# DmitryUlyanov/deep-image-prior

Hardware: AMD Instinct MI355X
Metric: optimisation iters/sec per image (skip-net 512x512 denoising) (higher is better)
Workload: dtype f32

## Files before the change

deep-image-prior_amd/csrc/bf3.h:

```cpp
#pragma once
#include "dip_common.h"

typedef __bf16 bf16x8 __attribute__((ext_vector_type(8)));
typedef unsigned u32x2 __attribute__((ext_vector_type(2)));
typedef unsigned u32x4 __attribute__((ext_vector_type(4)));

__device__ __forceinline__ void dip_bf3_split(float a, unsigned& h, unsigned& m, unsigned& l) {
    const unsigned uh = __float_as_uint(a) & 0xFFFF0000u;
    const float r1 = a - __uint_as_float(uh);
    const unsigned um = __float_as_uint(r1) & 0xFFFF0000u;
    const float r2 = r1 - __uint_as_float(um);
    h = uh;
    m = um;
    l = __float_as_uint(r2) & 0xFFFF0000u;
}

__device__ __forceinline__ unsigned dip_bf3_pack2(unsigned x0, unsigned x1) { return (x0 >> 16) | x1; }
__device__ __forceinline__ u32x2 dip_bf3_pack4(const unsigned (&x)[4]) {
    return u32x2{dip_bf3_pack2(x[0], x[1]), dip_bf3_pack2(x[2], x[3])};
}

template <int TR>
__device__ __forceinline__ f32x4 dip_bf3_transform(f32x4 v, const float* a4p, const float* b4p, float slope) {
    if constexpr (TR != 0) {
        const f32x4 a4 = *reinterpret_cast<const f32x4*>(a4p), b4 = *reinterpret_cast<const f32x4*>(b4p);
#pragma unroll
        for (int e = 0; e < 4; ++e) {
            const float tv = fmaf(a4[e], v[e], b4[e]);
            v[e] = TR == 1 ? dip_act_leaky(tv, slope) : dip_act(tv, slope);
        }
    }
    return v;
}

template <int NT, class F>
__device__ __forceinline__ void dip_bf3_products(F&& f) {
    dip_static_for<0, 5>([&](auto S) {
        constexpr int sm = 4 - decltype(S)::value;
        if constexpr (!((NT == 6 && sm > 2) || (NT == 8 && sm > 3))) {
            dip_static_for<0, 3>([&](auto PA) {
                constexpr int pa = decltype(PA)::value, pb = sm - pa;
                if constexpr (pb >= 0 && pb <= 2) f(PA, std::integral_constant<int, pb>{});
            });
        }
    });
}

static inline int dip_bf3_tr(const DipTransform& tr) { return tr.a == nullptr ? 0 : (tr.slope > 0.f ? 1 : 2); }
template <class F>
int dip_bf3_dispatch(int nt, int tr, F&& f) {
    auto with_nt = [&](auto NT) {
        if (tr == 0) return f(NT, std::integral_constant<int, 0>{});
        if (tr == 1) return f(NT, std::integral_constant<int, 1>{});
        return f(NT, std::integral_constant<int, 2>{});
    };
    if (nt == 6) return with_nt(std::integral_constant<int, 6>{});
    if (nt == 8) return with_nt(std::integral_constant<int, 8>{});
    return with_nt(std::integral_constant<int, 9>{});
}
```

deep-image-prior_amd/csrc/wgrad_bf3.hip:

```cpp
#include "dip_common.h"
#include "dip_group.h"
#include "bf3.h"
#include <stdlib.h>

namespace {

#ifdef DIP_W3_PROFILE
__device__ unsigned long long g_w3_prof[1024 * 8 * 8];
__device__ int g_w3_mode;
#define W3_T() __builtin_amdgcn_s_memtime()
#define W3_ADD(slot, t0, t1) prof[slot] += (t1) - (t0)
#else
#define W3_T() 0ull
#define W3_ADD(slot, t0, t1) ((void)0)
#endif

struct W3Cfg {
    static constexpr int TH = 2, TW = 16;
    static constexpr int HTH = TH + 2, HTW = TW + 2;
    static constexpr int U_ROW = 48;
    static constexpr int U_CH = HTH * U_ROW + 16;
    static constexpr int U_PLANE = 32 * U_CH;
    static constexpr int D_ROW = 32;
    static constexpr int D_CH = TH * D_ROW + 16;
    static constexpr int D_PLANE = 128 * D_CH;
    static constexpr int U_PAIRS = HTH * 9 * 8;
    static constexpr int D_PAIRS = TH * 8 * 32;
    static constexpr int U_SLOTS = 2, D_SLOTS = 2;
    static constexpr int LDS_BYTES = 3 * U_PLANE + 3 * D_PLANE + 2 * 512 * 4;
};

__device__ __forceinline__ void w3_store_planes(unsigned char* base, const unsigned (&h)[2][4], const unsigned (&m)[2][4], const unsigned (&l)[2][4],
                                                int ch_pitch, int plane_pitch) {
#pragma unroll
    for (int e = 0; e < 4; ++e) {
        *reinterpret_cast<unsigned*>(base + e * ch_pitch) = dip_bf3_pack2(h[0][e], h[1][e]);
        *reinterpret_cast<unsigned*>(base + e * ch_pitch + plane_pitch) = dip_bf3_pack2(m[0][e], m[1][e]);
        *reinterpret_cast<unsigned*>(base + e * ch_pitch + 2 * plane_pitch) = dip_bf3_pack2(l[0][e], l[1][e]);
    }
}
template <int NT>
__device__ __forceinline__ void w3_taps_of_row(const u32x4 (&w0)[3], const unsigned (&w1)[3], const bf16x8 (&b)[3], f32x16& acc0,
                                               f32x16& acc1, f32x16& acc2) {
    bf16x8 a[3][3];
#pragma unroll
    for (int p = 0; p < 3; ++p) {
        a[0][p] = __builtin_bit_cast(bf16x8, w0[p]);
        a[1][p] = __builtin_bit_cast(bf16x8, u32x4{__builtin_amdgcn_alignbyte(w0[p][1], w0[p][0], 2), __builtin_amdgcn_alignbyte(w0[p][2], w0[p][1], 2),
                                                     __builtin_amdgcn_alignbyte(w0[p][3], w0[p][2], 2), __builtin_amdgcn_alignbyte(w1[p], w0[p][3], 2)});
        a[2][p] = __builtin_bit_cast(bf16x8, u32x4{w0[p][1], w0[p][2], w0[p][3], w1[p]});
    }
    dip_bf3_products<NT>([&](auto PA, auto PB) {
        constexpr int pa = decltype(PA)::value, pb = decltype(PB)::value;
        acc0 = __builtin_amdgcn_mfma_f32_32x32x16_bf16(a[0][pa], b[pb], acc0, 0, 0, 0);
        __builtin_amdgcn_sched_barrier(0x7F6);
        acc1 = __builtin_amdgcn_mfma_f32_32x32x16_bf16(a[1][pa], b[pb], acc1, 0, 0, 0);
        __builtin_amdgcn_sched_barrier(0x7F6);
        acc2 = __builtin_amdgcn_mfma_f32_32x32x16_bf16(a[2][pa], b[pb], acc2, 0, 0, 0);
        __builtin_amdgcn_sched_barrier(0x7F6);
    });
}

template <int NT, int TR>
__global__ __launch_bounds__(256, 2) void wgrad_bf3_v1_kernel(const DipWgradDesc d, const int ntx, const int ntiles, const int CinP,
                                                              const int CoutP) {
    using C = W3Cfg;
    extern __shared__ __attribute__((aligned(16))) unsigned char smem[];
    unsigned char* Us = smem;
    unsigned char* Ds = smem + 3 * C::U_PLANE;
    float* tra = reinterpret_cast<float*>(Ds + 3 * C::D_PLANE);
    float* trb = tra + 512;

    const int tid = threadIdx.x, lane = tid & 63, l31 = lane & 31, half = lane >> 5;
    const int wave = __builtin_amdgcn_readfirstlane(tid >> 6);
    const int walker = blockIdx.x, nwalk = gridDim.x;
    const int c0 = blockIdx.y * 32;
    const int o0 = blockIdx.z * 128;
    const bool wave_active = (o0 + wave * 32) < CoutP;
    const bool do_bias = d.bias_partial != nullptr && blockIdx.y == 0;
    const float slope = d.tr.slope;

    if (TR) {
        for (int c = tid; c < 32; c += 256) {
            const bool ok = c0 + c < d.Cin;
            tra[c] = ok ? d.tr.a[c0 + c] : 1.f;
            trb[c] = ok ? d.tr.b[c0 + c] : 0.f;
        }
    }
    for (int i = tid; i < (3 * C::U_PLANE + 3 * C::D_PLANE) / 4; i += 256) reinterpret_cast<unsigned*>(smem)[i] = 0u;

    f32x16 acc[9];
#pragma unroll
    for (int t = 0; t < 9; ++t)
#pragma unroll
        for (int r = 0; r < 16; ++r) acc[t][r] = 0.f;
    float bs[2][4] = {{0.f, 0.f, 0.f, 0.f}, {0.f, 0.f, 0.f, 0.f}};

    f32x4 ur[C::U_SLOTS][2], dr[C::D_SLOTS][2];
    auto fetch = [&](int tile) {
        const int ty = tile / ntx, tx = tile - ty * ntx;
#pragma unroll
        for (int i = 0; i < C::U_SLOTS; ++i) {
            const int s = tid + i * 256;
            const int cg = s / 36, rem = s - cg * 36, hr = rem / 9, pp = rem - hr * 9;
            const int c = c0 + cg * 4;
            const int sr = dip_map_src(ty * C::TH + hr - d.off, d.Hin, d.pad_mode);
            const bool okc = s < C::U_PAIRS && c < d.Cin && sr >= 0;
#pragma unroll
            for (int q = 0; q < 2; ++q) {
                const int sc = dip_map_src(tx * C::TW + 2 * pp + q - d.off, d.Win, d.pad_mode);
                const bool ok = okc && sc >= 0;
                ur[i][q] = *reinterpret_cast<const f32x4*>(d.x + ((size_t)(ok ? sr : 0) * d.Win + (ok ? sc : 0)) * d.Cx + (ok ? c : 0));
            }
        }
#pragma unroll
        for (int i = 0; i < C::D_SLOTS; ++i) {
            const int s = tid + i * 256;
            const int cg = s >> 4, rem = s & 15, r = rem >> 3, pp = rem & 7;
            const int o = o0 + cg * 4;
            const int oy = ty * C::TH + r;
#pragma unroll
            for (int q = 0; q < 2; ++q) {
                const int ox = tx * C::TW + 2 * pp + q;
                const bool ok = oy < d.Hout && ox < d.Wout && o < d.Cdy;
                dr[i][q] = *reinterpret_cast<const f32x4*>(d.dy + ((size_t)(ok ? oy : 0) * d.Wout + (ok ? ox : 0)) * d.Cdy + (ok ? o : 0));
            }
        }
    };
    auto commit = [&](int tile) {
        const int ty = tile / ntx, tx = tile - ty * ntx;
#pragma unroll
        for (int i = 0; i < C::U_SLOTS; ++i) {
            const int s = tid + i * 256;
            if (s < C::U_PAIRS) {
                const int cg = s / 36, rem = s - cg * 36, hr = rem / 9, pp = rem - hr * 9;
                const int c = c0 + cg * 4;
                const int sr = dip_map_src(ty * C::TH + hr - d.off, d.Hin, d.pad_mode);
                unsigned h[2][4], m[2][4], l[2][4];
#pragma unroll
                for (int q = 0; q < 2; ++q) {
                    const int sc = dip_map_src(tx * C::TW + 2 * pp + q - d.off, d.Win, d.pad_mode);
                    const bool ok = c < d.Cin && sr >= 0 && sc >= 0;
                    f32x4 v = ur[i][q];
                    if (TR) {
                        const f32x4 a4 = *reinterpret_cast<const f32x4*>(tra + cg * 4), b4 = *reinterpret_cast<const f32x4*>(trb + cg * 4);
#pragma unroll
                        for (int e = 0; e < 4; ++e) {
                            const float tv = fmaf(a4[e], v[e], b4[e]);
                            v[e] = TR == 1 ? dip_act_leaky(tv, slope) : dip_act(tv, slope);
                        }
                    }
#pragma unroll
                    for (int e = 0; e < 4; ++e) dip_bf3_split(ok ? v[e] : 0.f, h[q][e], m[q][e], l[q][e]);
                }
                w3_store_planes(Us + (cg * 4) * C::U_CH + hr * C::U_ROW + pp * 4, h, m, l, C::U_CH, C::U_PLANE);
            }
        }
#pragma unroll
        for (int i = 0; i < C::D_SLOTS; ++i) {
            const int s = tid + i * 256;
            const int cg = s >> 4, rem = s & 15, r = rem >> 3, pp = rem & 7;
            const int o = o0 + cg * 4;
            const int oy = ty * C::TH + r;
            unsigned h[2][4], m[2][4], l[2][4];
#pragma unroll
            for (int q = 0; q < 2; ++q) {
                const int ox = tx * C::TW + 2 * pp + q;
                const bool ok = oy < d.Hout && ox < d.Wout && o < d.Cdy;
#pragma unroll
                for (int e = 0; e < 4; ++e) {
                    const float v = ok ? dr[i][q][e] : 0.f;
                    bs[i][e] += v;
                    dip_bf3_split(v, h[q][e], m[q][e], l[q][e]);
                }
            }
            w3_store_planes(Ds + (cg * 4) * C::D_CH + r * C::D_ROW + pp * 4, h, m, l, C::D_CH, C::D_PLANE);
        }
    };

    const unsigned char* ua = Us + l31 * C::U_CH + 16 * half;
    const unsigned char* da = Ds + (wave * 32 + l31) * C::D_CH + 16 * half;

    __syncthreads();
    if (walker < ntiles) fetch(walker);
    for (int tile = walker; tile < ntiles; tile += nwalk) {
        __syncthreads();
        commit(tile);
        __syncthreads();
        if (tile + nwalk < ntiles) fetch(tile + nwalk);
        if (wave_active) {
#pragma unroll
            for (int s = 0; s < 2; ++s) {
                bf16x8 b[3];
#pragma unroll
                for (int p = 0; p < 3; ++p) b[p] = *reinterpret_cast<const bf16x8*>(da + p * C::D_PLANE + s * C::D_ROW);
#pragma unroll
                for (int ky = 0; ky < 3; ++ky) {
                    const int hr = s + ky;
                    u32x4 w0[3];
                    unsigned w1[3];
#pragma unroll
                    for (int p = 0; p < 3; ++p) {
                        w0[p] = *reinterpret_cast<const u32x4*>(ua + p * C::U_PLANE + hr * C::U_ROW);
                        w1[p] = *reinterpret_cast<const unsigned*>(ua + p * C::U_PLANE + hr * C::U_ROW + 16);
                    }
#pragma unroll
                    for (int kx = 0; kx < 3; ++kx) {
                        bf16x8 a[3];
#pragma unroll
                        for (int p = 0; p < 3; ++p) {
                            u32x4 v;
                            if (kx == 0) v = w0[p];
                            else if (kx == 2) v = u32x4{w0[p][1], w0[p][2], w0[p][3], w1[p]};
                            else v = u32x4{__builtin_amdgcn_alignbyte(w0[p][1], w0[p][0], 2), __builtin_amdgcn_alignbyte(w0[p][2], w0[p][1], 2),
                                           __builtin_amdgcn_alignbyte(w0[p][3], w0[p][2], 2), __builtin_amdgcn_alignbyte(w1[p], w0[p][3], 2)};
                            a[p] = __builtin_bit_cast(bf16x8, v);
                        }
                        const int t = ky * 3 + kx;
                        dip_bf3_products<NT>([&](auto PA, auto PB) {
                            acc[t] = __builtin_amdgcn_mfma_f32_32x32x16_bf16(a[decltype(PA)::value], b[decltype(PB)::value], acc[t], 0, 0, 0);
                        });
                    }
                    __builtin_amdgcn_sched_barrier(0);
                }
            }
        }
    }

    if (wave_active) {
        const int o = o0 + wave * 32 + l31;
#pragma unroll
        for (int t = 0; t < 9; ++t)
#pragma unroll
            for (int r = 0; r < 16; ++r) {
                const int c = c0 + (r & 3) + 8 * (r >> 2) + 4 * half;
                if (c < CinP) d.partial[(((size_t)walker * 9 + t) * CinP + c) * CoutP + o] = acc[t][r];
            }
    }
    if (do_bias) {
        __syncthreads();
        float* red = reinterpret_cast<float*>(smem);
#pragma unroll
        for (int i = 0; i < C::D_SLOTS; ++i)
#pragma unroll
            for (int e = 0; e < 4; ++e) red[(tid + i * 256) * 4 + e] = bs[i][e];
        __syncthreads();
        if (tid < 128 && o0 + tid < CoutP) {
            const int cg = tid >> 2, e = tid & 3;
            float sum = 0.f;
            for (int k = 0; k < 16; ++k) sum += red[(cg * 16 + k) * 4 + e];
            d.bias_partial[(size_t)walker * CoutP + o0 + tid] = sum;
        }
    }
}

template <int NT, int TR>
int w3_launch_v1(const DipWgradDesc& d, hipStream_t st) {
    using C = W3Cfg;
    auto kern = wgrad_bf3_v1_kernel<NT, TR>;
    static bool attr_set[16] = {};
    if (dip_once_per_device(attr_set)) {
        hipError_t e = hipFuncSetAttribute(reinterpret_cast<const void*>(kern), hipFuncAttributeMaxDynamicSharedMemorySize, 160 * 1024);
        if (e != hipSuccess) { dip_set_error(hipGetErrorString(e)); return (int)e; }
    }
    const int ntx = dip_cdiv(d.Wout, C::TW), nty = dip_cdiv(d.Hout, C::TH);
    const int CinP = dip_round_up(d.Cin, 32), CoutP = dip_round_up(d.Cout, 32);
    const int nfull = ((d.Cin & 31) >= 1 && (d.Cin & 31) <= 4 && d.Cin > 32) ? (d.Cin >> 5) : dip_cdiv(d.Cin, 32);
    dip_launch(kern, dim3(d.nsplit, nfull, dip_cdiv(CoutP, 128)), dim3(256), C::LDS_BYTES, st, d, ntx, ntx * nty, CinP, CoutP);
    DIP_CHECK_LAUNCH();
    return 0;
}


template <int NT, int TR>
__global__ __launch_bounds__(512) void wgrad_bf3_kernel(const DipWgradDesc d, const int ntx, const int ntiles, const int CinP,
                                                        const int CoutP, const int c_end) {
    using C = W3Cfg;
    constexpr int U_PLANE2 = 64 * C::U_CH;
    constexpr int BUF = 3 * U_PLANE2 + 3 * C::D_PLANE;
    extern __shared__ __attribute__((aligned(16))) unsigned char smem[];
    float* tra = reinterpret_cast<float*>(smem + 2 * BUF);
    float* trb = tra + 64;

    const int tid = threadIdx.x, lane = tid & 63, l31 = lane & 31, half = lane >> 5;
    const int wave = __builtin_amdgcn_readfirstlane(tid >> 6);
    const int grp = wave >> 2, wq = wave & 3, tg = tid & 255;
    const int walker = blockIdx.x, nwalk = gridDim.x;
    const int c0 = blockIdx.y * 64 + grp * 32;
    const int o0 = blockIdx.z * 128;
    const bool wave_active = (o0 + wq * 32) < CoutP;
    const bool do_bias = d.bias_partial != nullptr && blockIdx.y == 0;
    const float slope = d.tr.slope;

    if (TR) {
        if (tid < 64) {
            const int c = blockIdx.y * 64 + tid;
            const bool ok = c < d.Cin;
            tra[tid] = ok ? d.tr.a[c] : 1.f;
            trb[tid] = ok ? d.tr.b[c] : 0.f;
        }
    }
    for (int i = tid; i < 2 * BUF / 4; i += 512) reinterpret_cast<unsigned*>(smem)[i] = 0u;

    f32x16 acc[9];
#pragma unroll
    for (int t = 0; t < 9; ++t)
#pragma unroll
        for (int r = 0; r < 16; ++r) acc[t][r] = 0.f;
    float bs[4] = {0.f, 0.f, 0.f, 0.f};

    int u_off[2], u_lds[2], u_hr[2], u_pp[2];
    bool u_valid[2];
#pragma unroll
    for (int i = 0; i < 2; ++i) {
        const int s = tg + i * 256;
        const int cg = s & 7, rem = s >> 3, hr = rem / 9, pp = rem - hr * 9;
        u_hr[i] = hr;
        u_pp[i] = pp;
        u_valid[i] = s < C::U_PAIRS && (c0 + cg * 4) < d.Cin;
        u_off[i] = u_valid[i] ? (hr * d.Win + 2 * pp) * d.Cx + c0 + cg * 4 : 0;
        u_lds[i] = (grp * 32 + cg * 4) * C::U_CH + hr * C::U_ROW + pp * 4;
    }
    const int u_c = c0 + (tg & 7) * 4;
    const int d_pp = tid & 7, d_r = (tid >> 6) & 1, d_cg = ((tid >> 7) << 3) | ((tid >> 3) & 7);
    const int d_o = o0 + d_cg * 4;
    const bool d_valid = d_o < d.Cdy;
    const int d_off = d_valid ? (d_r * d.Wout + 2 * d_pp) * d.Cdy + d_o : 0;
    const int d_lds = 3 * U_PLANE2 + (d_cg * 4) * C::D_CH + d_r * C::D_ROW + d_pp * 4;
    auto interior = [&](int ty, int tx) {
        return ty * C::TH - d.off >= 0 && ty * C::TH + C::HTH - 1 - d.off < d.Hin && tx * C::TW - d.off >= 0 &&
               tx * C::TW + C::HTW - 1 - d.off < d.Win && ty * C::TH + C::TH - 1 < d.Hout && tx * C::TW + C::TW - 1 < d.Wout;
    };

    f32x4 ur[2][2], dr[2];
    auto fetch = [&](int tile) {
        const int ty = tile / ntx, tx = tile - ty * ntx;
        const float* pu[2][2];
        const float* pd[2];
        if (interior(ty, tx)) {
            const float* bx = d.x + ((size_t)(ty * C::TH - d.off) * d.Win + (tx * C::TW - d.off)) * d.Cx;
            const float* by = d.dy + ((size_t)(ty * C::TH) * d.Wout + tx * C::TW) * d.Cdy;
#pragma unroll
            for (int i = 0; i < 2; ++i) {
                pu[i][0] = bx + u_off[i];
                pu[i][1] = pu[i][0] + d.Cx;
            }
            pd[0] = by + d_off;
            pd[1] = pd[0] + d.Cdy;
        } else {
#pragma unroll
            for (int i = 0; i < 2; ++i) {
                const int sr = dip_map_src(ty * C::TH + u_hr[i] - d.off, d.Hin, d.pad_mode);
                const bool okc = u_valid[i] && sr >= 0;
#pragma unroll
                for (int q = 0; q < 2; ++q) {
                    const int sc = dip_map_src(tx * C::TW + 2 * u_pp[i] + q - d.off, d.Win, d.pad_mode);
                    const bool ok = okc && sc >= 0;
                    pu[i][q] = d.x + ((size_t)(ok ? sr : 0) * d.Win + (ok ? sc : 0)) * d.Cx + (ok ? u_c : 0);
                }
            }
            const int oy = ty * C::TH + d_r;
#pragma unroll
            for (int q = 0; q < 2; ++q) {
                const int ox = tx * C::TW + 2 * d_pp + q;
                const bool ok = oy < d.Hout && ox < d.Wout && d_valid;
                pd[q] = d.dy + ((size_t)(ok ? oy : 0) * d.Wout + (ok ? ox : 0)) * d.Cdy + (ok ? d_o : 0);
            }
        }
#pragma unroll
        for (int i = 0; i < 2; ++i)
#pragma unroll
            for (int q = 0; q < 2; ++q) ur[i][q] = *reinterpret_cast<const f32x4*>(pu[i][q]);
#pragma unroll
        for (int q = 0; q < 2; ++q) dr[q] = *reinterpret_cast<const f32x4*>(pd[q]);
    };
    auto commit = [&](int tile, int buf) {
        const int ty = tile / ntx, tx = tile - ty * ntx;
        unsigned char* Bs = smem + buf * BUF;
        bool oku[2][2], okd[2];
        if (interior(ty, tx)) {
#pragma unroll
            for (int i = 0; i < 2; ++i) oku[i][0] = oku[i][1] = u_valid[i];
            okd[0] = okd[1] = d_valid;
        } else {
#pragma unroll
            for (int i = 0; i < 2; ++i) {
                const int sr = dip_map_src(ty * C::TH + u_hr[i] - d.off, d.Hin, d.pad_mode);
#pragma unroll
                for (int q = 0; q < 2; ++q) {
                    const int sc = dip_map_src(tx * C::TW + 2 * u_pp[i] + q - d.off, d.Win, d.pad_mode);
                    oku[i][q] = u_valid[i] && sr >= 0 && sc >= 0;
                }
            }
            const int oy = ty * C::TH + d_r;
#pragma unroll
            for (int q = 0; q < 2; ++q) okd[q] = oy < d.Hout && (tx * C::TW + 2 * d_pp + q) < d.Wout && d_valid;
        }
#pragma unroll
        for (int i = 0; i < 2; ++i) {
            if (tg + i * 256 < C::U_PAIRS) {
                unsigned h[2][4], m[2][4], l[2][4];
#pragma unroll
                for (int q = 0; q < 2; ++q) {
                    f32x4 v = ur[i][q];
                    v = dip_bf3_transform<TR>(v, tra + grp * 32 + (tg & 7) * 4, trb + grp * 32 + (tg & 7) * 4, slope);
#pragma unroll
                    for (int e = 0; e < 4; ++e) dip_bf3_split(oku[i][q] ? v[e] : 0.f, h[q][e], m[q][e], l[q][e]);
                }
                w3_store_planes(Bs + u_lds[i], h, m, l, C::U_CH, U_PLANE2);
            }
        }
        {
            unsigned h[2][4], m[2][4], l[2][4];
#pragma unroll
            for (int q = 0; q < 2; ++q) {
#pragma unroll
                for (int e = 0; e < 4; ++e) {
                    const float v = okd[q] ? dr[q][e] : 0.f;
                    bs[e] += v;
                    dip_bf3_split(v, h[q][e], m[q][e], l[q][e]);
                }
            }
            w3_store_planes(Bs + d_lds, h, m, l, C::D_CH, C::D_PLANE);
        }
    };

    const int ua_off = (grp * 32 + l31) * C::U_CH + 16 * half;
    const int da_off = 3 * U_PLANE2 + (wq * 32 + l31) * C::D_CH + 16 * half;
    auto mfma_tile = [&](int buf) {
        const unsigned char* ua = smem + buf * BUF + ua_off;
        const unsigned char* da = smem + buf * BUF + da_off;
        bf16x8 b[2][3];
#pragma unroll
        for (int s = 0; s < 2; ++s)
#pragma unroll
            for (int p = 0; p < 3; ++p) b[s][p] = *reinterpret_cast<const bf16x8*>(da + p * C::D_PLANE + s * C::D_ROW);
        u32x4 w0[2][3];
        unsigned w1[2][3];
#pragma unroll
        for (int p = 0; p < 3; ++p) {
            w0[0][p] = *reinterpret_cast<const u32x4*>(ua + p * U_PLANE2);
            w1[0][p] = *reinterpret_cast<const unsigned*>(ua + p * U_PLANE2 + 16);
        }
#pragma unroll
        for (int hr = 0; hr < 4; ++hr) {
            const int cur = hr & 1, nxt = cur ^ 1;
            if (hr < 3) {
#pragma unroll
                for (int p = 0; p < 3; ++p) {
                    w0[nxt][p] = *reinterpret_cast<const u32x4*>(ua + p * U_PLANE2 + (hr + 1) * C::U_ROW);
                    w1[nxt][p] = *reinterpret_cast<const unsigned*>(ua + p * U_PLANE2 + (hr + 1) * C::U_ROW + 16);
                }
            }
#pragma unroll
            for (int s = 0; s < 2; ++s) {
                const int ky = hr - s;
                if (ky < 0 || ky > 2) continue;
                w3_taps_of_row<NT>(w0[cur], w1[cur], b[s], acc[ky * 3], acc[ky * 3 + 1], acc[ky * 3 + 2]);
            }
            __builtin_amdgcn_sched_barrier(0);
        }
    };

#ifdef DIP_W3_PROFILE
    unsigned long long prof[8] = {0, 0, 0, 0, 0, 0, 0, 0};
#endif
    const unsigned long long tk0 = W3_T();
#ifdef DIP_W3_PROFILE
    const unsigned long long tr0 = __builtin_amdgcn_s_memrealtime();
    const int w3_mode = __builtin_amdgcn_readfirstlane(g_w3_mode);
#else
    constexpr int w3_mode = 0;
#endif
    __syncthreads();
    const int ntl = walker < ntiles ? (ntiles - 1 - walker) / nwalk + 1 : 0;
    if (ntl > 0) {
        fetch(walker);
        commit(walker, 0);
        if (ntl > 1) fetch(walker + nwalk);
    }
    __syncthreads();
    for (int h = 0; h < 2 * ntl; ++h) {
        const int kt = h >> 1, buf = kt & 1;
        const unsigned long long t0 = W3_T();
        if ((h & 1) == grp) {
            if (wave_active && w3_mode != 1) {
                __builtin_amdgcn_s_setprio(2);
                mfma_tile(buf);
                __builtin_amdgcn_s_setprio(0);
            }
            const unsigned long long t1 = W3_T();
            __syncthreads();
            W3_ADD(0, t0, t1);
            W3_ADD(1, t1, W3_T());
        } else {
            unsigned long long t1 = t0, t2 = t0;
            if (kt + 1 < ntl && w3_mode != 2) {
                commit(walker + (kt + 1) * nwalk, buf ^ 1);
                t1 = W3_T();
                if (kt + 2 < ntl) fetch(walker + (kt + 2) * nwalk);
                t2 = W3_T();
            }
            __syncthreads();
            W3_ADD(2, t0, t1);
            W3_ADD(3, t1, t2);
            W3_ADD(4, t2, W3_T());
        }
#ifdef DIP_W3_PROFILE
        prof[5] += 1;
#endif
    }
#ifdef DIP_W3_PROFILE
    prof[6] = W3_T() - tk0;
    prof[7] = __builtin_amdgcn_s_memrealtime() - tr0;
    if (lane == 0) {
        const int wg = (blockIdx.z * gridDim.y + blockIdx.y) * gridDim.x + blockIdx.x;
        if (wg < 1024)
            for (int i = 0; i < 8; ++i) g_w3_prof[(wg * 8 + wave) * 8 + i] = prof[i];
    }
#endif

    if (wave_active && c0 < c_end) {
        const int o = o0 + wq * 32 + l31;
#pragma unroll
        for (int t = 0; t < 9; ++t)
#pragma unroll
            for (int r = 0; r < 16; ++r) {
                const int c = c0 + (r & 3) + 8 * (r >> 2) + 4 * half;
                if (c < CinP) d.partial[(((size_t)walker * 9 + t) * CinP + c) * CoutP + o] = acc[t][r];
            }
    }
    if (do_bias) {
        float* red = reinterpret_cast<float*>(smem);
#pragma unroll
        for (int e = 0; e < 4; ++e) red[tid * 4 + e] = bs[e];
        __syncthreads();
        if (tid < 128 && o0 + tid < CoutP) {
            const int cg = tid >> 2, e = tid & 3;
            float sum = 0.f;
            for (int k = 0; k < 16; ++k) sum += red[((k & 7) + 8 * (cg & 7) + 64 * (k >> 3) + 128 * (cg >> 3)) * 4 + e];
            d.bias_partial[(size_t)walker * CoutP + o0 + tid] = sum;
        }
    }
}

template <int NT, int TR>
int w3_launch(const DipWgradDesc& d, hipStream_t st) {
    using C = W3Cfg;
    constexpr int LDS2 = 2 * (3 * 64 * C::U_CH + 3 * C::D_PLANE) + 2 * 64 * 4;
    auto kern = wgrad_bf3_kernel<NT, TR>;
    static bool attr_set[16] = {};
    if (dip_once_per_device(attr_set)) {
        hipError_t e = hipFuncSetAttribute(reinterpret_cast<const void*>(kern), hipFuncAttributeMaxDynamicSharedMemorySize, 160 * 1024);
        if (e != hipSuccess) { dip_set_error(hipGetErrorString(e)); return (int)e; }
    }
    const int ntx = dip_cdiv(d.Wout, C::TW), nty = dip_cdiv(d.Hout, C::TH);
    const int CinP = dip_round_up(d.Cin, 32), CoutP = dip_round_up(d.Cout, 32);
    const int nfull = ((d.Cin & 31) >= 1 && (d.Cin & 31) <= 4 && d.Cin > 32) ? (d.Cin >> 5) : dip_cdiv(d.Cin, 32);
    const bool has_tail = (d.Cin & 31) >= 1 && (d.Cin & 31) <= 4 && d.Cin > 32;
    dip_launch(kern, dim3(d.nsplit, dip_cdiv(nfull, 2), dip_cdiv(CoutP, 128)), dim3(512), LDS2, st, d, ntx, ntx * nty, CinP, CoutP,
               has_tail ? nfull * 32 : CinP);
    DIP_CHECK_LAUNCH();
    return 0;
}

}

#ifdef DIP_W3_PROFILE
extern "C" int dip_w3_prof_mode(int mode) { return (int)hipMemcpyToSymbol(HIP_SYMBOL(g_w3_mode), &mode, sizeof(int)); }
extern "C" int dip_w3_prof_read(unsigned long long* host, int n) {
    return (int)hipMemcpyFromSymbol(host, HIP_SYMBOL(g_w3_prof), (size_t)n * sizeof(unsigned long long));
}
#endif

extern "C" int dip_conv_bf3_terms(void);
extern "C" int dip_conv_wgrad_tail(const DipWgradDesc* dp, void* stream);

extern "C" int dip_wgrad_bf3_eligible(const DipWgradDesc* dp) {
    const DipWgradDesc& d = *dp;
    static const bool off = getenv("DIP_WGRAD_NO_BF3") != nullptr;
    if (off || dip_conv_bf3_terms() == 0) return 0;
    if (d.ks != 3 || d.stride != 1 || d.Cin < 32 || d.Cout < 97 || d.tap_groups > 1) return 0;
    if ((d.Cx & 3) || (d.Cdy & 3) || (d.tr.a != nullptr && d.Cin > 512)) return 0;
    const int tail = d.Cin & 31;
    if (tail >= 1 && tail <= 4 && (d.Cin >> 5) > 8) return 0;
    const int ntiles = dip_cdiv(d.Wout, 16) * dip_cdiv(d.Hout, 2);
    if (d.nsplit < 1 || d.nsplit > dip_cdiv(d.Wout, 16) * dip_cdiv(d.Hout, 4)) return 0;
    return ntiles >= 512 ? 1 : 0;
}

extern "C" int dip_wgrad_bf3(const DipWgradDesc* dp, void* stream) {
    const DipWgradDesc& d = *dp;
    hipStream_t st = reinterpret_cast<hipStream_t>(stream);
    const int nt = dip_conv_bf3_terms();
    if (nt == 0) DIP_FAIL("wgrad_bf3: the bf16-pipe arithmetic is switched off (DIP_CONV_BF3=0)");
    static const int v1_mode = [] { const char* e = getenv("DIP_WGRAD_BF3_V1"); return e ? atoi(e) : 0; }();
    const bool v1 = v1_mode == 1 || (v1_mode == 2 && dip_cdiv(d.Wout, 16) * dip_cdiv(d.Hout, 2) < 2048);
    const int rc = dip_bf3_dispatch(nt, dip_bf3_tr(d.tr), [&](auto NT, auto TR) {
        constexpr int T = decltype(NT)::value, R = decltype(TR)::value;
        return v1 ? w3_launch_v1<T, R>(d, st) : w3_launch<T, R>(d, st);
    });
    if (rc) return rc;
    if ((d.Cin & 31) >= 1 && (d.Cin & 31) <= 4 && d.Cin > 32) return dip_conv_wgrad_tail(dp, stream);
    return 0;
}
```

Baseline: 184.7.

## Restructure wgrad bf3 staging: recompute slot indices, split halo row loads, use perm packing

The staging of x and dy tiles into LDS is reorganised. The old two-iteration loop, which left lanes idle on the halo, is replaced by one full f32x4 slot per thread plus a scalar 'mini' slot that loads the last halo row on waves 2 and up. Per-thread slot offsets are now recomputed in each fetch and commit behind an asm barrier, so they are not held in registers across the MFMA loop. Offsets become 32-bit byte offsets, with a new eligibility guard against overflow. bf16 packing now uses v_perm, and the low term's mask is dropped because perm selects only the upper bytes. This aims to cut register pressure and VALU work in the staging path, at the cost of repeated index arithmetic.

```diff
diff --git a/deep-image-prior_amd/csrc/bf3.h b/deep-image-prior_amd/csrc/bf3.h
--- a/deep-image-prior_amd/csrc/bf3.h
+++ b/deep-image-prior_amd/csrc/bf3.h
@@ -12,14 +12,45 @@
     const float r2 = r1 - __uint_as_float(um);
     h = uh;
     m = um;
-    l = __float_as_uint(r2) & 0xFFFF0000u;
+    l = __float_as_uint(r2);
+}
+__device__ __forceinline__ void dip_bf3_split2(f32x2 a, u32x2& h, u32x2& m, u32x2& l) {
+#pragma unroll
+    for (int e = 0; e < 2; ++e) {
+        unsigned he, me, le;
+        dip_bf3_split(a[e], he, me, le);
+        h[e] = he;
+        m[e] = me;
+        l[e] = le;
+    }
+}
+__device__ __forceinline__ void dip_bf3_split4(f32x4 a, u32x4& h, u32x4& m, u32x4& l) {
+#pragma unroll
+    for (int e = 0; e < 4; ++e) {
+        unsigned he, me, le;
+        dip_bf3_split(a[e], he, me, le);
+        h[e] = he;
+        m[e] = me;
+        l[e] = le;
+    }
 }
 
-__device__ __forceinline__ unsigned dip_bf3_pack2(unsigned x0, unsigned x1) { return (x0 >> 16) | x1; }
+__device__ __forceinline__ unsigned dip_bf3_pack2(unsigned x0, unsigned x1) { return __builtin_amdgcn_perm(x1, x0, 0x07060302u); }
 __device__ __forceinline__ u32x2 dip_bf3_pack4(const unsigned (&x)[4]) {
     return u32x2{dip_bf3_pack2(x[0], x[1]), dip_bf3_pack2(x[2], x[3])};
 }
 
+template <int TR>
+__device__ __forceinline__ f32x2 dip_bf3_transform2(f32x2 v, f32x2 a2, f32x2 b2, float slope) {
+    if constexpr (TR != 0) {
+#pragma unroll
+        for (int e = 0; e < 2; ++e) {
+            const float tv = fmaf(a2[e], v[e], b2[e]);
+            v[e] = TR == 1 ? dip_act_leaky(tv, slope) : dip_act(tv, slope);
+        }
+    }
+    return v;
+}
 template <int TR>
 __device__ __forceinline__ f32x4 dip_bf3_transform(f32x4 v, const float* a4p, const float* b4p, float slope) {
     if constexpr (TR != 0) {
diff --git a/deep-image-prior_amd/csrc/wgrad_bf3.hip b/deep-image-prior_amd/csrc/wgrad_bf3.hip
--- a/deep-image-prior_amd/csrc/wgrad_bf3.hip
+++ b/deep-image-prior_amd/csrc/wgrad_bf3.hip
@@ -38,6 +38,19 @@
         *reinterpret_cast<unsigned*>(base + e * ch_pitch + plane_pitch) = dip_bf3_pack2(m[0][e], m[1][e]);
         *reinterpret_cast<unsigned*>(base + e * ch_pitch + 2 * plane_pitch) = dip_bf3_pack2(l[0][e], l[1][e]);
     }
+}
+__device__ __forceinline__ void w3_store_planes(unsigned char* base, const u32x4 (&h)[2], const u32x4 (&m)[2], const u32x4 (&l)[2], int ch_pitch,
+                                                int plane_pitch) {
+#pragma unroll
+    for (int e = 0; e < 4; ++e) {
+        *reinterpret_cast<unsigned*>(base + e * ch_pitch) = dip_bf3_pack2(h[0][e], h[1][e]);
+        *reinterpret_cast<unsigned*>(base + e * ch_pitch + plane_pitch) = dip_bf3_pack2(m[0][e], m[1][e]);
+        *reinterpret_cast<unsigned*>(base + e * ch_pitch + 2 * plane_pitch) = dip_bf3_pack2(l[0][e], l[1][e]);
+    }
+}
+__device__ __forceinline__ unsigned w3_here(unsigned v) {
+    asm volatile("" : "+v"(v));
+    return v;
 }
 template <int NT>
 __device__ __forceinline__ void w3_taps_of_row(const u32x4 (&w0)[3], const unsigned (&w1)[3], const bf16x8 (&b)[3], f32x16& acc0,
@@ -309,119 +322,145 @@
         for (int r = 0; r < 16; ++r) acc[t][r] = 0.f;
     float bs[4] = {0.f, 0.f, 0.f, 0.f};
 
-    int u_off[2], u_lds[2], u_hr[2], u_pp[2];
-    bool u_valid[2];
-#pragma unroll
-    for (int i = 0; i < 2; ++i) {
-        const int s = tg + i * 256;
-        const int cg = s & 7, rem = s >> 3, hr = rem / 9, pp = rem - hr * 9;
-        u_hr[i] = hr;
-        u_pp[i] = pp;
-        u_valid[i] = s < C::U_PAIRS && (c0 + cg * 4) < d.Cin;
-        u_off[i] = u_valid[i] ? (hr * d.Win + 2 * pp) * d.Cx + c0 + cg * 4 : 0;
-        u_lds[i] = (grp * 32 + cg * 4) * C::U_CH + hr * C::U_ROW + pp * 4;
-    }
-    const int u_c = c0 + (tg & 7) * 4;
-    const int d_pp = tid & 7, d_r = (tid >> 6) & 1, d_cg = ((tid >> 7) << 3) | ((tid >> 3) & 7);
-    const int d_o = o0 + d_cg * 4;
-    const bool d_valid = d_o < d.Cdy;
-    const int d_off = d_valid ? (d_r * d.Wout + 2 * d_pp) * d.Cdy + d_o : 0;
-    const int d_lds = 3 * U_PLANE2 + (d_cg * 4) * C::D_CH + d_r * C::D_ROW + d_pp * 4;
+    const bool mini = wq >= 2;
+    struct Slots {
+        int u_c, u_hr, u_pp, u_lds, m_c, m_pp, m_lds, d_o, d_r, d_pp, d_lds, tr_u, tr_m;
+        bool u_valid, m_valid, d_valid;
+        unsigned u_off, m_off, d_off;
+    };
+    auto slots = [&](unsigned t) {
+        Slots k;
+        const int g = t & 255, rem = g >> 3;
+        k.u_hr = rem / 9;
+        k.u_pp = rem - k.u_hr * 9;
+        k.m_pp = 5 + ((g >> 5) & 3);
+        k.tr_u = grp * 32 + (g & 7) * 4;
+        k.tr_m = grp * 32 + (g & 31);
+        k.u_c = c0 + (g & 7) * 4;
+        k.m_c = c0 + (g & 31);
+        k.u_valid = k.u_c < d.Cin;
+        k.m_valid = (c0 + (g & 28)) < d.Cin;
+        k.u_off = k.u_valid ? ((k.u_hr * d.Win + 2 * k.u_pp) * d.Cx + k.u_c) * 4u : 0u;
+        k.m_off = k.m_valid ? ((3 * d.Win + 2 * k.m_pp) * d.Cx + k.m_c) * 4u : 0u;
+        k.u_lds = k.tr_u * C::U_CH + k.u_hr * C::U_ROW + k.u_pp * 4;
+        k.m_lds = k.tr_m * C::U_CH + 3 * C::U_ROW + k.m_pp * 4;
+        const int d_cg = ((t >> 7) << 3) | ((t >> 3) & 7);
+        k.d_r = (t >> 6) & 1;
+        k.d_pp = t & 7;
+        k.d_o = o0 + d_cg * 4;
+        k.d_valid = k.d_o < d.Cdy;
+        k.d_off = k.d_valid ? ((k.d_r * d.Wout + 2 * k.d_pp) * d.Cdy + k.d_o) * 4u : 0u;
+        k.d_lds = 3 * U_PLANE2 + (d_cg * 4) * C::D_CH + k.d_r * C::D_ROW + k.d_pp * 4;
+        return k;
+    };
     auto interior = [&](int ty, int tx) {
         return ty * C::TH - d.off >= 0 && ty * C::TH + C::HTH - 1 - d.off < d.Hin && tx * C::TW - d.off >= 0 &&
                tx * C::TW + C::HTW - 1 - d.off < d.Win && ty * C::TH + C::TH - 1 < d.Hout && tx * C::TW + C::TW - 1 < d.Wout;
     };
-
-    f32x4 ur[2][2], dr[2];
+    auto border_u = [&](int ty, int tx, int hr, int pp, bool valid, int c, size_t (&o)[2], bool (&ok)[2]) {
+        const int sr = dip_map_src(ty * C::TH + hr - d.off, d.Hin, d.pad_mode);
+#pragma unroll
+        for (int q = 0; q < 2; ++q) {
+            const int sc = dip_map_src(tx * C::TW + 2 * pp + q - d.off, d.Win, d.pad_mode);
+            ok[q] = valid && sr >= 0 && sc >= 0;
+            o[q] = ok[q] ? ((size_t)sr * d.Win + sc) * d.Cx + c : 0;
+        }
+    };
+    auto border_d = [&](int ty, int tx, const Slots& k, size_t (&o)[2], bool (&ok)[2]) {
+        const int oy = ty * C::TH + k.d_r;
+#pragma unroll
+        for (int q = 0; q < 2; ++q) {
+            const int ox = tx * C::TW + 2 * k.d_pp + q;
+            ok[q] = oy < d.Hout && ox < d.Wout && k.d_valid;
+            o[q] = ok[q] ? ((size_t)oy * d.Wout + ox) * d.Cdy + k.d_o : 0;
+        }
+    };
+
+    f32x4 ur[2], dr[2];
+    f32x2 mr = {0.f, 0.f};
     auto fetch = [&](int tile) {
         const int ty = tile / ntx, tx = tile - ty * ntx;
-        const float* pu[2][2];
-        const float* pd[2];
+        const Slots k = slots(w3_here(tid));
         if (interior(ty, tx)) {
-            const float* bx = d.x + ((size_t)(ty * C::TH - d.off) * d.Win + (tx * C::TW - d.off)) * d.Cx;
-            const float* by = d.dy + ((size_t)(ty * C::TH) * d.Wout + tx * C::TW) * d.Cdy;
-#pragma unroll
-            for (int i = 0; i < 2; ++i) {
-                pu[i][0] = bx + u_off[i];
-                pu[i][1] = pu[i][0] + d.Cx;
-            }
-            pd[0] = by + d_off;
-            pd[1] = pd[0] + d.Cdy;
+            const char* bx = reinterpret_cast<const char*>(d.x + ((size_t)(ty * C::TH - d.off) * d.Win + (tx * C::TW - d.off)) * d.Cx);
+            const char* by = reinterpret_cast<const char*>(d.dy + ((size_t)(ty * C::TH) * d.Wout + tx * C::TW) * d.Cdy);
+#pragma unroll
+            for (int q = 0; q < 2; ++q) ur[q] = *reinterpret_cast<const f32x4*>(bx + (size_t)q * d.Cx * 4 + k.u_off);
+            if (mini) {
+#pragma unroll
+                for (int q = 0; q < 2; ++q) mr[q] = *reinterpret_cast<const float*>(bx + (size_t)q * d.Cx * 4 + k.m_off);
+            }
+#pragma unroll
+            for (int q = 0; q < 2; ++q) dr[q] = *reinterpret_cast<const f32x4*>(by + (size_t)q * d.Cdy * 4 + k.d_off);
         } else {
-#pragma unroll
-            for (int i = 0; i < 2; ++i) {
-                const int sr = dip_map_src(ty * C::TH + u_hr[i] - d.off, d.Hin, d.pad_mode);
-                const bool okc = u_valid[i] && sr >= 0;
-#pragma unroll
-                for (int q = 0; q < 2; ++q) {
-                    const int sc = dip_map_src(tx * C::TW + 2 * u_pp[i] + q - d.off, d.Win, d.pad_mode);
-                    const bool ok = okc && sc >= 0;
-                    pu[i][q] = d.x + ((size_t)(ok ? sr : 0) * d.Win + (ok ? sc : 0)) * d.Cx + (ok ? u_c : 0);
-                }
-            }
-            const int oy = ty * C::TH + d_r;
-#pragma unroll
-            for (int q = 0; q < 2; ++q) {
-                const int ox = tx * C::TW + 2 * d_pp + q;
-                const bool ok = oy < d.Hout && ox < d.Wout && d_valid;
-                pd[q] = d.dy + ((size_t)(ok ? oy : 0) * d.Wout + (ok ? ox : 0)) * d.Cdy + (ok ? d_o : 0);
-            }
-        }
-#pragma unroll
-        for (int i = 0; i < 2; ++i)
-#pragma unroll
-            for (int q = 0; q < 2; ++q) ur[i][q] = *reinterpret_cast<const f32x4*>(pu[i][q]);
-#pragma unroll
-        for (int q = 0; q < 2; ++q) dr[q] = *reinterpret_cast<const f32x4*>(pd[q]);
+            size_t ou[2], om[2], od[2];
+            bool ok[2];
+            border_u(ty, tx, k.u_hr, k.u_pp, k.u_valid, k.u_c, ou, ok);
+            border_d(ty, tx, k, od, ok);
+#pragma unroll
+            for (int q = 0; q < 2; ++q) ur[q] = *reinterpret_cast<const f32x4*>(d.x + ou[q]);
+            if (mini) {
+                border_u(ty, tx, 3, k.m_pp, k.m_valid, k.m_c, om, ok);
+#pragma unroll
+                for (int q = 0; q < 2; ++q) mr[q] = d.x[om[q]];
+            }
+#pragma unroll
+            for (int q = 0; q < 2; ++q) dr[q] = *reinterpret_cast<const f32x4*>(d.dy + od[q]);
+        }
     };
     auto commit = [&](int tile, int buf) {
         const int ty = tile / ntx, tx = tile - ty * ntx;
         unsigned char* Bs = smem + buf * BUF;
-        bool oku[2][2], okd[2];
+        const Slots k = slots(w3_here(tid));
+        bool oku[2], okm[2], okd[2];
         if (interior(ty, tx)) {
-#pragma unroll
-            for (int i = 0; i < 2; ++i) oku[i][0] = oku[i][1] = u_valid[i];
-            okd[0] = okd[1] = d_valid;
+            oku[0] = oku[1] = k.u_valid;
+            okm[0] = okm[1] = k.m_valid;
+            okd[0] = okd[1] = k.d_valid;
         } else {
-#pragma unroll
-            for (int i = 0; i < 2; ++i) {
-                const int sr = dip_map_src(ty * C::TH + u_hr[i] - d.off, d.Hin, d.pad_mode);
-#pragma unroll
-                for (int q = 0; q < 2; ++q) {
-                    const int sc = dip_map_src(tx * C::TW + 2 * u_pp[i] + q - d.off, d.Win, d.pad_mode);
-                    oku[i][q] = u_valid[i] && sr >= 0 && sc >= 0;
+            size_t o[2];
+            border_u(ty, tx, k.u_hr, k.u_pp, k.u_valid, k.u_c, o, oku);
+            border_u(ty, tx, 3, k.m_pp, k.m_valid, k.m_c, o, okm);
+            border_d(ty, tx, k, o, okd);
+        }
+        {
+            u32x4 h[2], m[2], l[2];
+#pragma unroll
+            for (int q = 0; q < 2; ++q) {
+                f32x4 v = dip_bf3_transform<TR>(ur[q], tra + k.tr_u, trb + k.tr_u, slope);
+#pragma unroll
+                for (int e = 0; e < 4; ++e) v[e] = oku[q] ? v[e] : 0.f;
+                dip_bf3_split4(v, h[q], m[q], l[q]);
+            }
+            w3_store_planes(Bs + k.u_lds, h, m, l, C::U_CH, U_PLANE2);
+        }
+        if (mini) {
+            f32x2 v = mr;
+            if (TR) {
+                const float ta = tra[k.tr_m], tb = trb[k.tr_m];
+                v = dip_bf3_transform2<TR>(v, f32x2{ta, ta}, f32x2{tb, tb}, slope);
+            }
+#pragma unroll
+            for (int q = 0; q < 2; ++q) v[q] = okm[q] ? v[q] : 0.f;
+            u32x2 h, m, l;
+            dip_bf3_split2(v, h, m, l);
+            *reinterpret_cast<unsigned*>(Bs + k.m_lds) = dip_bf3_pack2(h[0], h[1]);
+            *reinterpret_cast<unsigned*>(Bs + k.m_lds + U_PLANE2) = dip_bf3_pack2(m[0], m[1]);
+            *reinterpret_cast<unsigned*>(Bs + k.m_lds + 2 * U_PLANE2) = dip_bf3_pack2(l[0], l[1]);
+        }
+        {
+            u32x4 h[2], m[2], l[2];
+#pragma unroll
+            for (int q = 0; q < 2; ++q) {
+                f32x4 v;
+#pragma unroll
+                for (int e = 0; e < 4; ++e) {
+                    v[e] = okd[q] ? dr[q][e] : 0.f;
+                    bs[e] += v[e];
                 }
-            }
-            const int oy = ty * C::TH + d_r;
-#pragma unroll
-            for (int q = 0; q < 2; ++q) okd[q] = oy < d.Hout && (tx * C::TW + 2 * d_pp + q) < d.Wout && d_valid;
-        }
-#pragma unroll
-        for (int i = 0; i < 2; ++i) {
-            if (tg + i * 256 < C::U_PAIRS) {
-                unsigned h[2][4], m[2][4], l[2][4];
-#pragma unroll
-                for (int q = 0; q < 2; ++q) {
-                    f32x4 v = ur[i][q];
-                    v = dip_bf3_transform<TR>(v, tra + grp * 32 + (tg & 7) * 4, trb + grp * 32 + (tg & 7) * 4, slope);
-#pragma unroll
-                    for (int e = 0; e < 4; ++e) dip_bf3_split(oku[i][q] ? v[e] : 0.f, h[q][e], m[q][e], l[q][e]);
-                }
-                w3_store_planes(Bs + u_lds[i], h, m, l, C::U_CH, U_PLANE2);
-            }
-        }
-        {
-            unsigned h[2][4], m[2][4], l[2][4];
-#pragma unroll
-            for (int q = 0; q < 2; ++q) {
-#pragma unroll
-                for (int e = 0; e < 4; ++e) {
-                    const float v = okd[q] ? dr[q][e] : 0.f;
-                    bs[e] += v;
-                    dip_bf3_split(v, h[q][e], m[q][e], l[q][e]);
-                }
-            }
-            w3_store_planes(Bs + d_lds, h, m, l, C::D_CH, C::D_PLANE);
+                dip_bf3_split4(v, h[q], m[q], l[q]);
+            }
+            w3_store_planes(Bs + k.d_lds, h, m, l, C::D_CH, C::D_PLANE);
         }
     };
 
@@ -582,6 +621,7 @@
     if (off || dip_conv_bf3_terms() == 0) return 0;
     if (d.ks != 3 || d.stride != 1 || d.Cin < 32 || d.Cout < 97 || d.tap_groups > 1) return 0;
     if ((d.Cx & 3) || (d.Cdy & 3) || (d.tr.a != nullptr && d.Cin > 512)) return 0;
+    if ((long long)d.Win * d.Cx * 16 >= (1ll << 32) || (long long)d.Wout * d.Cdy * 8 >= (1ll << 32)) return 0;
     const int tail = d.Cin & 31;
     if (tail >= 1 && tail <= 4 && (d.Cin >> 5) > 8) return 0;
     const int ntiles = dip_cdiv(d.Wout, 16) * dip_cdiv(d.Hout, 2);
```

Measured after the change: 185.2, median of 6. No clear change (+0.3%).
